# Lemok00/IDEAS

Hardware: AMD Instinct MI355X
Metric: train images/sec at 256x256 (G+D+Ex step) (higher is better)
Workload: dtype f32; 1 GPU; IDEAS N=1 sigma=1 256x256 batch=32/GPU full G+D+Ex iteration (lazy R1 every 16, EMA), full-width nets, HIP kernels (BASELINE.json configs[2]); global_batch=32, parallelism=dp1, r1_steps_in_window=0, ranks=1

## Files before the change

### ideas_amd/_lib.py

```python
from __future__ import annotations

import ctypes as C
import os
from typing import Optional

import torch

_HERE = os.path.dirname(os.path.abspath(__file__))
LIB_PATH = os.environ.get("IDEAS_HIP_LIB", os.path.join(_HERE, "libideas_hip.so"))

NCHW, NHWC = 0, 1
F32 = 0
F32_B3 = 1
BF16 = 2
F16 = 3
F64 = 4


def act_dtype(t: torch.Tensor) -> int:
    if t.dtype == torch.float32:
        return F32
    if t.dtype == torch.bfloat16:
        return BF16
    raise RuntimeError(f"ideas_amd: only float32 and bfloat16 activations are implemented, got {t.dtype}")
# ... 28 lines not shown
                ("block0", C.c_int), ("nblocks", C.c_int), ("pad_", C.c_int)]


PREP_B3_SPLIT, PREP_B3_WINO, PREP_BF16_PACK = 0, 1, 2


class LinearSeg(C.Structure):
    _fields_ = [("w", C.c_void_p), ("bias", C.c_void_p), ("y", C.c_void_p), ("gw", C.c_void_p), ("gb", C.c_void_p),
                ("n", C.c_int), ("ldw", C.c_int), ("ldy", C.c_int), ("ldgw", C.c_int), ("scale", C.c_float), ("bias_mul", C.c_float),
                ("tile0", C.c_int), ("pad_", C.c_int)]


LINEAR_MAX_SEGMENTS = 32
MBSTD_MAX_PARTIALS = 64
NOISE_ACT_MAX_PARTIALS = 2048
LPIPS_MAX_PARTIALS = 64
POOL_MAX_S2, POOL_MAX_S1P1, POOL_AVG_S1P1_VALID = 0, 1, 2
FEATURE_STATS_MAX_DIM = 4096
PATH_LERP, PATH_SLERP, PATH_MAX_DIM = 0, 1, 4096

_P = C.c_void_p
_PROTOS = {
    "ideas_abi_version": (C.c_int, []),
    "ideas_sizeof_conv_params": (C.c_int, []),
    "ideas_strerror": (C.c_char_p, [C.c_int]),
    "ideas_stream_create": (C.c_int, [C.POINTER(C.c_void_p), C.c_int]),
    "ideas_stream_destroy": (C.c_int, [_P]),
    "ideas_fused_bias_act": (C.c_int, [_P, _P, _P, _P, _P, C.c_int64, C.c_int, C.c_int64, C.c_int, C.c_int, C.c_int,
                                       C.c_float, C.c_float, C.c_int, _P]),
    "ideas_upfirdn2d": (C.c_int, [_P, _P, _P] + [C.c_int] * 14 + [C.c_float, C.c_int, C.c_int, C.c_int, _P]),
    "ideas_fir_up2_add": (C.c_int, [_P, _P, _P, _P] + [C.c_int] * 8 + [C.c_float, C.c_int, C.c_int, _P]),
    "ideas_blur_fused": (C.c_int, [_P, _P, _P] + [C.c_int] * 8 + [C.c_float, C.c_int, C.c_int, _P, _P, _P, C.c_float, C.c_float,
                                   C.c_int, _P]),
    "ideas_conv_igemm": (C.c_int, [_P, _P, _P, _P, _P, _P, _P, C.POINTER(ConvParams), C.c_int, _P]),
    "ideas_conv_igemm_multi": (C.c_int, [C.c_int, _P, _P, C.POINTER(C.c_void_p), _P, _P, C.POINTER(ConvParams), C.c_int, _P]),
    "ideas_b3_conv_supported": (C.c_int, [C.POINTER(ConvParams)]),
    "ideas_b3_wgrad_supported": (C.c_int, [C.POINTER(ConvParams)]),
    "ideas_b3_wgrad3_supported": (C.c_int, [C.POINTER(ConvParams)]),
    "ideas_b3_wino_supported": (C.c_int, [C.POINTER(ConvParams)]),
    "ideas_b3_wino_split_weights": (C.c_int, [_P, _P, C.c_int, C.c_int, C.c_int64, C.c_int64, C.c_int64, C.c_int64, C.c_int64, _P]),
    "ideas_b3_split_weights": (C.c_int, [_P, _P, C.c_int, C.c_int, C.c_int, _P]),
    "ideas_b3_split_weights_strided": (C.c_int, [_P, _P] + [C.c_int] * 4 + [C.c_int64] * 4 + [_P]),
    "ideas_bf16_conv_supported": (C.c_int, [C.POINTER(ConvParams), C.c_int]),
    "ideas_bf16_wgrad_supported": (C.c_int, [C.POINTER(ConvParams), C.c_int]),
    "ideas_bf16_direct_supported": (C.c_int, [C.POINTER(ConvParams)]),
    "ideas_bf16_pack_weights": (C.c_int, [_P, _P, _P, C.c_int, C.c_int, C.c_int, C.c_int, _P]),
    "ideas_bf16_pack_weights_strided": (C.c_int, [_P, _P, _P] + [C.c_int] * 5 + [C.c_int64] * 4 + [_P]),
    "ideas_conv3x3_wino": (C.c_int, [_P, _P, _P, _P, _P, _P, _P, C.POINTER(ConvParams), C.c_int, _P]),
    "ideas_conv3x3_wino_wgrad": (C.c_int, [_P, _P, _P, _P, _P, C.POINTER(ConvParams), C.c_int, _P]),
    "ideas_wino_wgrad_fold": (C.c_int, [_P, _P, C.c_int, C.c_int] + [C.c_int64] * 4 + [C.c_int, _P]),
    "ideas_b3_blur_conv_s2_supported": (C.c_int, [C.POINTER(ConvParams), C.c_int, C.c_int, C.c_int]),
    "ideas_b3_blur_conv_s2": (C.c_int, [_P, _P, _P, _P, C.POINTER(C.c_float), C.POINTER(C.c_float), _P, _P, C.POINTER(ConvParams),
                                        C.c_int, C.c_int, C.c_int, _P]),
    "ideas_b3_blur_conv_s2_mod": (C.c_int, [_P, _P, _P, _P, C.POINTER(C.c_float), C.POINTER(C.c_float), _P, _P, _P, _P,
                                            C.POINTER(ConvParams), C.c_int, C.c_int, C.c_int, _P]),
    "ideas_conv_direct": (C.c_int, [_P, _P, _P, _P, _P, _P, _P, C.POINTER(ConvParams), C.c_int, _P]),
    "ideas_conv_wgrad": (C.c_int, [_P, _P, _P, _P, _P, C.POINTER(ConvParams), C.c_int, _P]),
    "ideas_conv_wgrad_direct": (C.c_int, [_P, _P, _P, _P, _P, C.POINTER(ConvParams), C.c_int, _P]),
    "ideas_demod": (C.c_int, [_P, _P, _P, C.c_int, C.c_int, C.c_int, C.c_float, _P]),
    "ideas_weight_sqsum": (C.c_int, [_P, _P] + [C.c_int] * 4 + [C.c_int64] * 4 + [C.c_float, _P]),
    "ideas_weight_sqsum_f64": (C.c_int, [_P, _P] + [C.c_int] * 4 + [C.c_int64] * 4 + [C.c_double, _P]),
    "ideas_demod_bwd": (C.c_int, [_P] * 7 + [C.c_int] * 3 + [C.c_float, _P]),
    "ideas_demod_wgrad": (C.c_int, [_P] * 4 + [C.c_int] * 5 + [C.c_int64] * 8 + [C.c_float, _P]),
    "ideas_pixel_dot": (C.c_int, [_P, _P, _P, C.c_int, C.c_int64, C.c_int, C.c_int, _P]),
    "ideas_reflect_fold": (C.c_int, [_P, _P, C.c_int, C.c_int, C.c_int, C.c_int, C.c_int, C.c_int, _P]),
    "ideas_adam_ema": (C.c_int, [_P, _P, _P, _P, C.c_int64, C.c_float, C.c_float, C.c_float, C.c_float, C.c_float, _P]),
# ... 99 lines not shown
```

### ideas_amd/csrc/upfirdn2d.hip

```cpp
#include "common.hpp"

namespace {

struct FirParams {
    int B, C, in_h, in_w, out_h, out_w, kh, kw;
    int up_x, up_y, down_x, down_y, pad_x0, pad_y0;
    float gain;
    int flip;
    int seg_rows;
};

#define GENERIC_TAP_LDS 32768
template <bool NHWC, typename T, typename A, typename K>
__global__ __launch_bounds__(256) void upfirdn2d_generic(T* __restrict__ y, const T* __restrict__ x,
                                                         const K* __restrict__ fir, FirParams p, int lds_taps) {
    extern __shared__ double s_taps[];
    A* sk = reinterpret_cast<A*>(s_taps);
    if (lds_taps) {
        for (int t = threadIdx.x; t < p.kh * p.kw; t += blockDim.x) {
            int ky = t / p.kw, kx = t % p.kw;
            int src = p.flip ? (p.kh - 1 - ky) * p.kw + (p.kw - 1 - kx) : t;
            sk[t] = (A)fir[src] * (A)p.gain;
        }
        __syncthreads();
// ... 368 lines not shown
            if (t > 0) { hb.x = fmaf(v[t].x, kh[t - 1], hb.x); hb.y = fmaf(v[t].y, kh[t - 1], hb.y); hb.z = fmaf(v[t].z, kh[t - 1], hb.z); hb.w = fmaf(v[t].w, kh[t - 1], hb.w); }
        }
    };
    auto vsum = [&](const float4& r0, const float4& r1, const float4& r2, const float4& r3) {
        return make_float4(r0.x * kv[0] + r1.x * kv[1] + r2.x * kv[2] + r3.x * kv[3], r0.y * kv[0] + r1.y * kv[1] + r2.y * kv[2] + r3.y * kv[3],
                           r0.z * kv[0] + r1.z * kv[1] + r2.z * kv[2] + r3.z * kv[3], r0.w * kv[0] + r1.w * kv[1] + r2.w * kv[2] + r3.w * kv[3]);
    };
    float4 a0, a1, a2, a3, a4, b0, b1, b2, b3, b4;
    {
        const int iy0 = oy0 - p.pad_y0;
        hrow(iy0 + 0, a0, b0); hrow(iy0 + 1, a1, b1); hrow(iy0 + 2, a2, b2);
    }
    int oy = oy0;
#pragma unroll 1
    for (; oy + 1 < oy1; oy += 2) {
        hrow(oy - p.pad_y0 + 3, a3, b3);
        hrow(oy - p.pad_y0 + 4, a4, b4);
        fin(oy, 0, vsum(a0, a1, a2, a3));
        if (colB) fin(oy, 1, vsum(b0, b1, b2, b3));
        fin(oy + 1, 0, vsum(a1, a2, a3, a4));
        if (colB) fin(oy + 1, 1, vsum(b1, b2, b3, b4));
        a0 = a2; a1 = a3; a2 = a4; b0 = b2; b1 = b3; b2 = b4;
    }
    if (oy < oy1) {
        hrow(oy - p.pad_y0 + 3, a3, b3);
        fin(oy, 0, vsum(a0, a1, a2, a3));
        if (colB) fin(oy, 1, vsum(b0, b1, b2, b3));
    }
    if (EPI == EPI_ACT_BWD) {
        const float part[4] = {bsum.x, bsum.y, bsum.z, bsum.w};
        bgrad_flush(s_bg, ep.bgrad, p.C, active, 4 * c4, part, 4);
    }
}
template <int EPI, typename E>
__global__ __launch_bounds__(256) void blur4_bf16x8_c2(uint4* __restrict__ y, const uint4* __restrict__ x,
                                                       const float* __restrict__ fir, FirParams p, FirEpi ep) {
    __shared__ float sk[16];
    extern __shared__ float s_bg[];
    blur4_c2<VecX8<E>, EPI>(y, x, fir, p, ep, sk, s_bg);
}

template <typename T, int EPI>
__global__ __launch_bounds__(256) void blur4_nhwc(typename T::raw* __restrict__ y, const typename T::raw* __restrict__ x,
                                                  const float* __restrict__ fir, FirParams p, FirEpi ep) {
    typedef typename T::raw raw;
    constexpr int N = T::N;
    __shared__ float sk[16];
    extern __shared__ float s_bg[];
    stage_taps(sk, fir, p);
    const int CV = p.C >> T::SHIFT;
    Tile tl;
    const bool active = decode_tile(tl, p, CV, p.out_w, p.out_h);
    if (EPI != EPI_ACT_BWD && !active) return;
    const int ox = tl.col, oy0 = tl.r0, oy1 = tl.r1;
    const int ix0 = ox - p.pad_x0;
    float k[16];
#pragma unroll
    for (int t = 0; t < 16; ++t) k[t] = sk[t];
    const raw* xb = x + (int64_t)tl.b * p.in_h * p.in_w * CV + tl.cv;
    raw* yb = y + (((int64_t)tl.b * p.out_h) * p.out_w + ox) * CV + tl.cv;
    const raw* rb = reinterpret_cast<const raw*>(ep.ref) + (((int64_t)tl.b * p.out_h) * p.out_w + ox) * CV + tl.cv;
    float bb[N] = {}, bsum[N] = {};
    if (EPI == EPI_BIAS_ACT) {
#pragma unroll
        for (int e = 0; e < N; ++e) bb[e] = ep.bias[N * tl.cv + e];
    }
// ... 265 lines not shown
        }
    }
    if (dtype == IDEAS_BF16 && p.C % 8 == 0)
        FIR_LAUNCH((blur4_bf16x8_c2<EPI, ideas_bf16>), pairs * (p.C / 8), lds, stream, (uint4*)y, (const uint4*)x, fir, p, ep);
    else if (dtype == IDEAS_BF16)
        FIR_LAUNCH((blur4_nhwc<VecBf16x4, EPI>), total, lds, stream, (ideas_bf16x4*)y, (const ideas_bf16x4*)x, fir, p, ep);
    else
        FIR_LAUNCH(blur4_f32_c2<EPI>, pairs * (p.C / 4), lds, stream, (float4*)y, (const float4*)x, fir, p, ep);
    return ideas_launch_status();
}

static void launch_down2(void* y, const void* x, const float* fir, const FirParams& p, int64_t tiles, int dtype, bool x8, hipStream_t stream) {
    if (x8 && dtype == IDEAS_F16)
        FIR_LAUNCH(fir4_down2_bf16x8<_Float16>, tiles * (p.C / 8), 0, stream, (uint4*)y, (const uint4*)x, fir, p);
    else if (x8)
        FIR_LAUNCH(fir4_down2_bf16x8<ideas_bf16>, tiles * (p.C / 8), 0, stream, (uint4*)y, (const uint4*)x, fir, p);
    else if (dtype == IDEAS_BF16)
        FIR_LAUNCH(fir4_down2_nhwc<VecBf16x4>, tiles * (p.C / 4), 0, stream, (ideas_bf16x4*)y, (const ideas_bf16x4*)x, fir, p);
    else
        FIR_LAUNCH(fir4_down2_nhwc<VecF32>, tiles * (p.C / 4), 0, stream, (float4*)y, (const float4*)x, fir, p);
}
static void launch_up2(void* y, const void* x, const float* fir, const FirParams& p, const void* resid, int64_t tiles, int dtype, bool x8,
                       hipStream_t stream) {
    if (x8 && dtype == IDEAS_F16)
        FIR_LAUNCH(fir4_up2<VecX8<_Float16>>, tiles * (p.C / 8), 0, stream, (uint4*)y, (const uint4*)x, fir, p, (const uint4*)resid);
    else if (x8)
        FIR_LAUNCH(fir4_up2<VecX8<ideas_bf16>>, tiles * (p.C / 8), 0, stream, (uint4*)y, (const uint4*)x, fir, p, (const uint4*)resid);
    else if (dtype == IDEAS_BF16)
        FIR_LAUNCH(fir4_up2<VecBf16x4>, tiles * (p.C / 4), 0, stream, (ideas_bf16x4*)y, (const ideas_bf16x4*)x, fir, p, (const ideas_bf16x4*)resid);
    else
        FIR_LAUNCH(fir4_up2<VecF32>, tiles * (p.C / 4), 0, stream, (float4*)y, (const float4*)x, fir, p, (const float4*)resid);
}

#undef FIR_LAUNCH

extern "C" int ideas_blur_fused(void* y, const void* x, const float* fir, int B, int C, int in_h, int in_w, int out_h, int out_w,
                                int pad_x0, int pad_y0, float gain, int flip, int mode, const void* ref, const float* bias,
                                float* bias_grad, float alpha, float scale, int dtype, void* stream_) {
    if (dtype != IDEAS_F32 && dtype != IDEAS_BF16) return IDEAS_E_UNSUPPORTED;
    if (!y || !x || !fir) return IDEAS_E_NULL;
    if (B <= 0 || C <= 0 || in_h <= 0 || in_w <= 0 || out_h <= 0 || out_w <= 0) return IDEAS_E_SHAPE;
    if (C % 4 || C > 8192) return IDEAS_E_UNSUPPORTED;
    if (!ideas_aligned16(x) || !ideas_aligned16(y)) return IDEAS_E_ALIGN;
    FirParams p{B, C, in_h, in_w, out_h, out_w, 4, 4, 1, 1, 1, 1, pad_x0, pad_y0, gain, flip, 16};
    FirEpi ep{ref, bias, bias_grad, alpha, scale};
    hipStream_t stream = (hipStream_t)stream_;
    if (mode == EPI_ACT_BWD) {
        if (!ref || !bias_grad) return IDEAS_E_NULL;
        if (!ideas_aligned16(ref)) return IDEAS_E_ALIGN;
        return launch_blur4<EPI_ACT_BWD>(y, x, fir, p, ep, dtype, stream);
    }
    if (mode == EPI_BIAS_ACT) {
        if (!bias) return IDEAS_E_NULL;
        if (!ideas_aligned16(bias)) return IDEAS_E_ALIGN;
        return launch_blur4<EPI_BIAS_ACT>(y, x, fir, p, ep, dtype, stream);
    }
    return IDEAS_E_UNSUPPORTED;
}

static int upfirdn2d_impl(void* y, const void* x, const float* fir, int B, int C, int in_h, int in_w, int out_h,
                          int out_w, int kh, int kw, int up_x, int up_y, int down_x, int down_y, int pad_x0,
                          int pad_y0, float gain, int flip, int layout, int dtype, void* stream_, const void* resid) {
    if (dtype != IDEAS_F32 && dtype != IDEAS_BF16 && dtype != IDEAS_F16 && dtype != IDEAS_F64) return IDEAS_E_UNSUPPORTED;
    if (dtype == IDEAS_BF16 && layout != IDEAS_NHWC) return IDEAS_E_UNSUPPORTED;
    if (!y || !x || !fir) return IDEAS_E_NULL;
    if (B <= 0 || C <= 0 || in_h <= 0 || in_w <= 0 || out_h <= 0 || out_w <= 0) return IDEAS_E_SHAPE;
    if (kh <= 0 || kw <= 0) return IDEAS_E_UNSUPPORTED;
// ... 85 lines not shown
```

### ideas_amd/op/modulated_conv.py

```python
from __future__ import annotations

import math
from typing import Optional

import torch
from torch.autograd import Function
from torch.autograd.function import once_differentiable

from .. import _lib
from ..precision import to_act, to_f32
from . import conv as _conv
from .conv import conv2d, conv_dgrad_raw, conv_fwd_raw, conv_transpose2d, conv_wgrad_raw, _nhwc
from .conv_plan import ConvGeom, convT_out_size
from . import conv_plan
from . import scratch
from .upfirdn2d import _geometry, blur_bias_act, blur_pads, upfirdn2d, upfirdn2d_raw
from .fused_act import bias_sink, fused_leaky_relu
from .grad_sink import weight_grad


def pixel_dot(a: torch.Tensor, g: torch.Tensor) -> torch.Tensor:
    a, g = _nhwc(a), _nhwc(g)
    b, c, h, w = a.shape
    out = scratch.zeros((b, c), a.device, torch.float64)
    if a.dtype != g.dtype:
        a, g = a.float(), g.float()
    if a.dtype == torch.bfloat16 and c % 4:
        a, g = a.float(), g.float()
    rc = _lib.load().ideas_pixel_dot(_lib.ptr(out), _lib.ptr(a), _lib.ptr(g), b, h * w, c, _lib.act_dtype(a), _lib.stream_ptr())
    _lib.check(rc, "ideas_pixel_dot")
    return out


def _weight_sqsum(w: torch.Tensor, scale: float, dtype, entry: str, key: str) -> torch.Tensor:
    def make():
        cout, cin, kh, kw = w.shape
        wsq = torch.empty((cout, cin), device=w.device, dtype=dtype)
        _lib.check(getattr(_lib.load(), entry)(_lib.ptr(wsq), _lib.ptr(w), cout, cin, kh, kw, *w.stride(), float(scale * scale),
                                               _lib.stream_ptr()), entry)
        return wsq
    return conv_plan.cached(w, (key, float(scale)), make)


def weight_sqsum(w: torch.Tensor, scale: float) -> torch.Tensor:
    return _weight_sqsum(w, scale, torch.float32, "ideas_weight_sqsum", "wsq")


def weight_sqsum_f64(w: torch.Tensor, scale: float) -> torch.Tensor:
    return _weight_sqsum(w, scale, torch.float64, "ideas_weight_sqsum_f64", "wsq64")
# ... 24 lines not shown
    cout = w.shape[0]
    if dot_s.dtype != torch.float64 or (dot_d is not None and dot_d.dtype != torch.float64):
        raise RuntimeError("_style_grads takes the float64 accumulators of pixel_dot / act_bwd_dot")
    if d is not None:
        gq, wsq = torch.empty_like(d), weight_sqsum_f64(w, gain)
    rc = _lib.load().ideas_demod_bwd(_lib.ptr(gs), _lib.ptr(gq), _lib.ptr(dot_s), _lib.ptr(dot_d), _lib.ptr(d), _lib.ptr(s),
                                     _lib.ptr(wsq), b, cin, cout, float(eps), _lib.stream_ptr())
    _lib.check(rc, "ideas_demod_bwd")
    return gs, gq


def _demod_wgrad(gw: torch.Tensor, w: torch.Tensor, gq: torch.Tensor, s: torch.Tensor, gain: float) -> None:
    cout, cin, kh, kw = w.shape
    rc = _lib.load().ideas_demod_wgrad(_lib.ptr(gw), _lib.ptr(w), _lib.ptr(gq), _lib.ptr(s), s.shape[0], cout, cin, kh, kw,
                                       *w.stride(), *gw.stride(), float(2.0 * gain * gain), _lib.stream_ptr())
    _lib.check(rc, "ideas_demod_wgrad")


def act_bwd_dot(gy: torch.Tensor, out: torch.Tensor, bias: torch.Tensor, alpha: float, act_gain: float, bias_grad_into=None):
    gy, out = _nhwc(gy), _nhwc(out)
    if gy.dtype != out.dtype:
        gy = gy.to(out.dtype)
    b, c, h, w = out.shape
    gpre = torch.empty_like(out)
    bg = bias_grad_into if bias_grad_into is not None else torch.zeros(c, device=out.device, dtype=torch.float32)
    dot = scratch.zeros((b, c), out.device, torch.float64)
    rc = _lib.load().ideas_act_bwd_dot(_lib.ptr(gpre), _lib.ptr(bg), _lib.ptr(dot), _lib.ptr(gy), _lib.ptr(out),
                                       _lib.ptr(bias), None, b, h * w, c, float(alpha), float(act_gain), _lib.act_dtype(out),
                                       _lib.stream_ptr())
    _lib.check(rc, "ideas_act_bwd_dot")
    return gpre, (None if bias_grad_into is not None else bg), dot


def _mod_geom(mode: str, k: int) -> ConvGeom:
    if mode == "same":
        return ConvGeom(k, k, 1, k // 2, False)
    return ConvGeom(k, k, 1 if (mode == "down" and k == 1) else 2, 0, False)


def _down_blur(x, fir, k: int, pad2):
    down = 2 if k == 1 else 1
    return (down,) + _geometry((x.shape[2], x.shape[3]), fir, 1, down, pad2)


def _mod_forward(x, w, s, d, mode: str, fir, pad2, gain: float, bias=None, slope: float = 0.2, act_gain: float = 1.0, resid=None,
                 want_xb: bool = False):
    k = w.shape[2]
    g = _mod_geom(mode, k)
    epi = dict(lin=s, lout=d, bias=bias, act=bias is not None, act_gain=act_gain, alpha=slope)
    if mode == "same":
        return conv_fwd_raw(x, w, g, gain, resid=resid, **epi), None
    if mode == "up":
        return conv_dgrad_raw(x, w.transpose(0, 1), g, convT_out_size(x.shape[2], x.shape[3], g), gain, lin=s, lout=d), None
    if k == 3 and _conv.mod_blur_conv_ok(x, w, fir, pad2, want_xb=want_xb):
        return _conv.blur_conv_s2_raw(x, w, fir, pad2, gain, want_xb=want_xb, **epi)
    down, pad4, bhw, _ = _down_blur(x, fir, k, pad2)
    xb = upfirdn2d_raw(x, fir, (1, 1), (down, down), pad4, bhw, flip=True)
    return conv_fwd_raw(xb, w, g, gain, **epi), xb


class _ModConv(Function):

    @staticmethod
    def forward(ctx, x, w, s, b, mode: str, fir, pad2, gain: float, demod: bool, eps: float, slope: float, act_gain: float):
        x = _nhwc(x)
        s = s.contiguous()
        ctx.bias_ref = b
        if b is not None:
            b = b.contiguous()
        d = demod_of(w, s, gain, eps) if demod else None
        need_w = ctx.needs_input_grad[1]
        y, xb = _mod_forward(x, w, s, d, mode, fir, pad2, gain, b, slope, act_gain, want_xb=need_w)
        ctx.mode, ctx.pad2, ctx.gain, ctx.eps, ctx.slope, ctx.act_gain = mode, pad2, gain, eps, slope, act_gain
        keep = dict(x=x, w=w, s=s, fir=fir, d=d, b=b,
                    y=y if (b is not None or d is not None) else None,
                    xb=xb if need_w else None)
        ctx.names = [n for n, t in keep.items() if t is not None]
        ctx.save_for_backward(*(keep[n] for n in ctx.names))
        return y

    @staticmethod
    @once_differentiable
    def backward(ctx, gy):
        t = dict(zip(ctx.names, ctx.saved_tensors))
        x, w, s, d, b, y = t["x"], t["w"], t["s"], t.get("d"), t.get("b"), t.get("y")
        mode, gain = ctx.mode, ctx.gain
        g = _mod_geom(mode, w.shape[2])
        need_x, need_w, need_s, need_b = ctx.needs_input_grad[:4]
        gb = dot_d = None
        if b is not None:
            gpre, gb, dot_d = act_bwd_dot(gy, y, b, ctx.slope, ctx.act_gain, bias_grad_into=bias_sink(ctx.bias_ref) if need_b else None)
        else:
            gpre = gy = _nhwc(gy)
        gx = gw = gs = gq = None
        if need_x or need_s:
            if mode == "up":
                gx = conv_fwd_raw(gpre, w.transpose(0, 1), g, gain, lin=d, lout=s)
            elif mode == "same":
                gx = conv_dgrad_raw(gpre, w, g, (x.shape[2], x.shape[3]), gain, lin=d, lout=s)
            else:
                down, _, bhw, g_pad = _down_blur(x, t["fir"], w.shape[2], ctx.pad2)
                gx = conv_dgrad_raw(gpre, w, g, bhw, gain, lin=d, lout=s)
                gx = upfirdn2d_raw(gx, t["fir"], (down, down), (1, 1), g_pad, (x.shape[2], x.shape[3]), flip=False)
        if need_s or (need_w and d is not None):
            dot_s = pixel_dot(x, gx) if need_s else scratch.zeros(tuple(s.shape), s.device, torch.float64)
            if d is not None and dot_d is None:
                dot_d = pixel_dot(gy, y)
            gs, gq = _style_grads(dot_s, dot_d, s, d, w, gain, ctx.eps)
        if need_w:
            xin = t["xb"] if mode == "down" else x

            def grad(out):
                if mode == "up":
                    r = conv_wgrad_raw(xin, gpre, g, (w.shape[1], w.shape[0], w.shape[2], w.shape[3]), gain, lin=d, lout=s,
                                       out=None if out is None else out.transpose(0, 1)).transpose(0, 1)
                else:
                    r = conv_wgrad_raw(gpre, xin, g, tuple(w.shape), gain, lin=s, lout=d, out=out)
                if gq is not None:
                    _demod_wgrad(r, w, gq, s, gain)
                return r
            gw = weight_grad(w, grad, gpre, xin, s, d, gq)
        return ((gx if need_x else None), gw, (gs if need_s else None), (gb if need_b else None),
                None, None, None, None, None, None, None, None)
# ... 35 lines not shown


def modulated_conv2d(x: torch.Tensor, weight: torch.Tensor, style: torch.Tensor, demodulate: bool = True,
                     upsample: bool = False, fir: Optional[torch.Tensor] = None, eps: float = 1e-8,
                     act_bias: Optional[torch.Tensor] = None, negative_slope: float = 0.2,
                     act_scale: float = 2 ** 0.5, resid: Optional[torch.Tensor] = None, downsample: bool = False) -> torch.Tensor:
    if upsample and downsample:
        raise ValueError("modulated_conv2d: upsample and downsample are exclusive")
    _lib.require_cuda(x, weight, style)
    mode = "down" if downsample else "up" if upsample else "same"
    if mode != "same" and fir is None:
        raise RuntimeError(f"modulated_conv2d({mode}sample=True) needs the blur FIR")
    if downsample:
        if resid is not None:
            raise RuntimeError("modulated_conv2d(resid=...) is the no-grad fast path of the fused same-resolution conv")
        _lib.require_cuda(fir, act_bias)
    x, style = to_act(x), to_f32(style)
    if resid is not None:
        resid = to_act(resid)
    w = weight[0] if weight.dim() == 5 else weight
    cout, cin, k, _ = w.shape
    if _SECOND_ORDER[0] and torch.is_grad_enabled() and resid is None:
        return _modulated_conv2d_composite(x, w, style, demodulate, upsample, fir, eps, act_bias, negative_slope, act_scale, downsample)
    scale = 1.0 / math.sqrt(cin * k * k)
    pad2 = blur_pads(fir.shape[0], k, up=upsample) if mode != "same" else None
    fuse_act = act_bias is not None and not upsample and demodulate and cout % 4 == 0
    if resid is not None:
        if not fuse_act or torch.is_grad_enabled():
            raise RuntimeError("modulated_conv2d(resid=...) is the no-grad fast path of the fused same-resolution conv")
        style = style.contiguous()
        d = demod_raw(style, weight_sqsum(w, scale), eps)
        return _mod_forward(x, w, style, d, mode, None, None, scale, act_bias.contiguous(), float(negative_slope), float(act_scale),
                            resid=resid)[0]
    y = _ModConv.apply(x, w, style, act_bias if fuse_act else None, mode, *((fir, pad2) if downsample else (None, None)),
                       scale, bool(demodulate), float(eps), float(negative_slope), float(act_scale))
    if upsample:
        if act_bias is not None:
            return blur_bias_act(y, fir, pad2, act_bias, negative_slope, act_scale)
        return upfirdn2d(y, fir, pad=pad2)
    if act_bias is not None and not fuse_act:
        y = fused_leaky_relu(y, act_bias, negative_slope, act_scale)
    return y
```

### ideas_amd/op/upfirdn2d.py

```python
from __future__ import annotations

from typing import Tuple

import torch
from torch.autograd import Function

from .. import _lib


def upfirdn2d_raw(x: torch.Tensor, fir: torch.Tensor, up: Tuple[int, int], down: Tuple[int, int],
                  pad: Tuple[int, int, int, int], out_hw: Tuple[int, int], flip: bool, gain: float = 1.0) -> torch.Tensor:
    _lib.require_cuda(x, fir)
    dt = _lib.op_dtype(x)
    if x.dim() != 4:
        raise RuntimeError("upfirdn2d expects a 4-D [B, C, H, W] tensor")
    lib = _lib.load()
    b, c, h, w = x.shape
    kh, kw = fir.shape
    oh, ow = out_hw
    if oh <= 0 or ow <= 0:
        raise RuntimeError(f"upfirdn2d: empty output {oh}x{ow}")
    if x.is_contiguous(memory_format=torch.channels_last):
        layout, fmt = _lib.NHWC, torch.channels_last
    elif x.is_contiguous() and dt != _lib.BF16:
# ... 10 lines not shown
    return y


BLUR_ACT_BWD, BLUR_BIAS_ACT = 1, 2


def blur_fused_ok(x: torch.Tensor, fir: torch.Tensor) -> bool:
    return (x.dim() == 4 and x.is_cuda and x.dtype in (torch.float32, torch.bfloat16) and x.shape[1] % 4 == 0 and tuple(fir.shape) == (4, 4)
            and x.is_contiguous(memory_format=torch.channels_last))


def blur_fused_raw(x: torch.Tensor, fir: torch.Tensor, pad: Tuple[int, int, int, int], out_hw: Tuple[int, int], flip: bool,
                   mode: int, ref=None, bias=None, bias_grad=None, alpha: float = 0.2, scale: float = 1.0) -> torch.Tensor:
    _lib.require_cuda(x, fir, ref, bias, bias_grad)
    b, c, h, w = x.shape
    oh, ow = out_hw
    x = x if x.is_contiguous(memory_format=torch.channels_last) else x.contiguous(memory_format=torch.channels_last)
    if ref is not None:
        if tuple(ref.shape) != (b, c, oh, ow):
            raise RuntimeError("blur_fused: ref shape mismatch")
        if ref.dtype != x.dtype:
            x = x.to(ref.dtype)
        ref = ref if ref.is_contiguous(memory_format=torch.channels_last) else ref.contiguous(memory_format=torch.channels_last)
    if bias is not None:
        bias = bias.contiguous().to(torch.float32)
    y = torch.empty((b, c, oh, ow), device=x.device, dtype=x.dtype, memory_format=torch.channels_last)
    rc = _lib.load().ideas_blur_fused(_lib.ptr(y), _lib.ptr(x), _lib.ptr(fir.contiguous().to(torch.float32)), b, c, h, w, oh, ow,
                                      pad[0], pad[2], 1.0, int(flip), mode, _lib.ptr(ref), _lib.ptr(bias), _lib.ptr(bias_grad),
                                      float(alpha), float(scale), _lib.act_dtype(x), _lib.stream_ptr())
    _lib.check(rc, "ideas_blur_fused")
    return y


def blur_geometry(in_hw: Tuple[int, int], fir: torch.Tensor, pad2: Tuple[int, int]):
    return _geometry(in_hw, fir, 1, 1, pad2)


class _BlurBiasAct(Function):

    @staticmethod
    def forward(ctx, x, fir, pad2, bias, slope: float, scale: float):
        pad4, out_hw, g_pad = blur_geometry((x.shape[2], x.shape[3]), fir, pad2)
        out = blur_fused_raw(x, fir, pad4, out_hw, True, BLUR_BIAS_ACT, bias=bias, alpha=slope, scale=scale)
        ctx.pad4, ctx.g_pad, ctx.in_size, ctx.out_hw, ctx.slope, ctx.scale = pad4, g_pad, tuple(x.shape), out_hw, slope, scale
        ctx.bias_ref = bias
        ctx.save_for_backward(out, fir)
        return out

    @staticmethod
    def backward(ctx, gy):
        from .fused_act import FusedLeakyReLUFunctionBackward, bias_act_raw, bias_sink
        out, fir = ctx.saved_tensors
        one = (1, 1)
        tgt = bias_sink(ctx.bias_ref) if ctx.needs_input_grad[3] else None
        if tgt is not None:
            g_pre, gb = bias_act_raw(gy, None, out, 1, ctx.slope, ctx.scale, bias_grad_into=tgt)
        else:
            g_pre, gb = FusedLeakyReLUFunctionBackward.apply(gy, out, ctx.slope, ctx.scale, True)
        gx = None
        if ctx.needs_input_grad[0]:
            gx = UpFirDn2dBackward.apply(g_pre, fir, one, one, ctx.pad4, ctx.g_pad, ctx.in_size, ctx.out_hw)
        return gx, None, None, (gb if (ctx.needs_input_grad[3] and tgt is None) else None), None, None


def blur_bias_act(x: torch.Tensor, fir: torch.Tensor, pad, bias: torch.Tensor, negative_slope: float = 0.2,
                  scale: float = 2 ** 0.5) -> torch.Tensor:
# ... 139 lines not shown
```

### include/ideas_hip.h

```cpp
#ifndef IDEAS_HIP_H
#define IDEAS_HIP_H

#include <stdint.h>

#ifdef __cplusplus
extern "C" {
#endif

#define IDEAS_ABI_VERSION 4

enum { IDEAS_NCHW = 0, IDEAS_NHWC = 1 };
enum { IDEAS_F32 = 0, IDEAS_F32_B3 = 1, IDEAS_BF16 = 2, IDEAS_F16 = 3, IDEAS_F64 = 4 };

enum {
    IDEAS_OK = 0,
    IDEAS_E_NULL = -1,
    IDEAS_E_SHAPE = -2,
    IDEAS_E_UNSUPPORTED = -3,
    IDEAS_E_ALIGN = -4
};

int ideas_abi_version(void);
int ideas_sizeof_conv_params(void);
const char* ideas_strerror(int code);

int ideas_stream_create(void** out_stream, int prio);
int ideas_stream_destroy(void* stream);

int ideas_fused_bias_act(void* y, const void* x, const void* b, const void* ref, float* bias_grad,
                         int64_t n, int C, int64_t inner, int layout,
                         int act, int grad, float alpha, float scale, int dtype, void* stream);

int ideas_channel_sum(float* out, const void* x, int64_t n, int C, int clear, int dtype, void* stream);

int ideas_upfirdn2d(void* y, const void* x, const float* fir,
                    int B, int C, int in_h, int in_w, int out_h, int out_w,
                    int kh, int kw, int up_x, int up_y, int down_x, int down_y,
                    int pad_x0, int pad_y0, float gain, int flip,
                    int layout, int dtype, void* stream);

int ideas_fir_up2_add(void* y, const void* x, const float* fir, const void* resid, int B, int C, int in_h, int in_w, int out_h,
                      int out_w, int pad_x0, int pad_y0, float gain, int flip, int dtype, void* stream);

#define IDEAS_BLUR_ACT_BWD 1
#define IDEAS_BLUR_BIAS_ACT 2
int ideas_blur_fused(void* y, const void* x, const float* fir, int B, int C, int in_h, int in_w, int out_h, int out_w,
                     int pad_x0, int pad_y0, float gain, int flip, int mode, const void* ref, const float* bias,
                     float* bias_grad, float alpha, float scale, int dtype, void* stream);

typedef struct ideas_conv_params {
    int B, IH, IW, Cin;
    int YH, YW, Cout;
    int OH, OW;
    int TY, TX;
    int sy, sx, dy, dx, offy, offx;
    int osy, osx, ooy, oox;
    int reflect;
    int act;
    float alpha, act_gain, resid_gain;
    int accumulate;
    float gain;
} ideas_conv_params;

int ideas_conv_igemm(void* y, const void* x, const void* wmat, const float* in_scale, const float* out_scale,
                     const float* bias, const void* resid, const ideas_conv_params* p, int dtype, void* stream);

int ideas_b3_conv_supported(const ideas_conv_params* p);
int ideas_b3_wgrad_supported(const ideas_conv_params* p);
int ideas_b3_wgrad3_supported(const ideas_conv_params* p);
int ideas_b3_split_weights(void* planes, const void* wmat, int Cout, int K, int Cin, void* stream);
int ideas_b3_split_weights_strided(void* planes, const float* w, int Cout, int TY, int TX, int Cin, int64_t sn, int64_t sty,
                                   int64_t stx, int64_t sc, void* stream);
int ideas_b3_wino_supported(const ideas_conv_params* p);
int ideas_b3_wino_split_weights(void* planes, const void* w, int N, int C, int64_t sn, int64_t sky, int64_t skx, int64_t sc,
                                int64_t base, void* stream);

int ideas_bf16_conv_supported(const ideas_conv_params* p, int scaled);
int ideas_bf16_wgrad_supported(const ideas_conv_params* p, int scaled);
int ideas_bf16_pack_weights(void* pack, const void* wmat, const float* in_scale, int B, int Cout, int K, int Cin, void* stream);
int ideas_bf16_pack_weights_strided(void* pack, const float* w, const float* in_scale, int B, int Cout, int TY, int TX, int Cin,
                                    int64_t sn, int64_t sty, int64_t stx, int64_t sc, void* stream);
// ... 154 lines not shown
```

Baseline: 81.50 images/sec.

## Fuse upsample modconv blur+bias-act backward with activation grad and demod dot

Result: no change. 82.15 images/sec (median of 6 runs) (+0.8%).

```diff
diff --git a/ideas_amd/_lib.py b/ideas_amd/_lib.py
--- a/ideas_amd/_lib.py
+++ b/ideas_amd/_lib.py
@@ -84,6 +84,7 @@
     "ideas_fir_up2_add": (C.c_int, [_P, _P, _P, _P] + [C.c_int] * 8 + [C.c_float, C.c_int, C.c_int, _P]),
     "ideas_blur_fused": (C.c_int, [_P, _P, _P] + [C.c_int] * 8 + [C.c_float, C.c_int, C.c_int, _P, _P, _P, C.c_float, C.c_float,
                                    C.c_int, _P]),
+    "ideas_act_bwd_blur": (C.c_int, [_P] * 7 + [C.c_int] * 8 + [C.c_float, C.c_float, C.c_int, _P]),
     "ideas_conv_igemm": (C.c_int, [_P, _P, _P, _P, _P, _P, _P, C.POINTER(ConvParams), C.c_int, _P]),
     "ideas_conv_igemm_multi": (C.c_int, [C.c_int, _P, _P, C.POINTER(C.c_void_p), _P, _P, C.POINTER(ConvParams), C.c_int, _P]),
     "ideas_b3_conv_supported": (C.c_int, [C.POINTER(ConvParams)]),
diff --git a/ideas_amd/csrc/upfirdn2d.hip b/ideas_amd/csrc/upfirdn2d.hip
--- a/ideas_amd/csrc/upfirdn2d.hip
+++ b/ideas_amd/csrc/upfirdn2d.hip
@@ -424,6 +424,156 @@
         bgrad_flush(s_bg, ep.bgrad, p.C, active, 4 * c4, part, 4);
     }
 }
+#define ACT_BLUR_SLOTS 2
+template <int PX>
+__global__ __launch_bounds__(256) void act_bwd_blur4_f32(float4* __restrict__ y, const float4* __restrict__ gy, const float4* __restrict__ ref,
+                                                         const float* __restrict__ fir, const float* __restrict__ bias,
+                                                         float* __restrict__ bgrad, double* __restrict__ dot, FirParams p, float alpha,
+                                                         float scale) {
+    __shared__ float sk[16];
+    extern __shared__ double s_red[];
+    double* s_dot = s_red;
+    float* s_bg = reinterpret_cast<float*>(s_red + ACT_BLUR_SLOTS * p.C);
+    for (int c = threadIdx.x; c < ACT_BLUR_SLOTS * p.C; c += blockDim.x) s_dot[c] = 0.0;
+    for (int c = threadIdx.x; c < p.C; c += blockDim.x) s_bg[c] = 0.f;
+    stage_taps(sk, fir, p);
+    float kh[4], kv[4];
+    const bool sep = factor_taps(sk, kh, kv);
+    const int C4 = p.C >> 2;
+    const int cols = (p.out_w + 1) >> 1;
+    Tile tl;
+    const bool active = decode_tile(tl, p, C4, cols, p.out_h);
+    const int c4 = tl.cv, b = tl.b, oy0 = tl.r0, oy1 = tl.r1;
+    const int b_first = (int)(((int64_t)blockIdx.x * blockDim.x) / ((int64_t)((p.out_h + p.seg_rows - 1) / p.seg_rows) * cols * C4));
+    const int ox = 2 * tl.col;
+    const bool colB = ox + 1 < p.out_w;
+    const int ix0 = ox - PX;
+    const float4 zero = make_float4(0.f, 0.f, 0.f, 0.f);
+    const float4* gb = gy + (int64_t)b * p.in_h * p.in_w * C4 + c4;
+    const float4* rb = ref + (int64_t)b * p.in_h * p.in_w * C4 + c4;
+    float4* yb = y + (((int64_t)b * p.out_h) * p.out_w + ox) * C4 + c4;
+    const float4 bb = bias ? *reinterpret_cast<const float4*>(bias + 4 * c4) : zero;
+    const float inv_gain = 1.0f / scale, inv_alpha = 1.0f / alpha;
+    float4 bsum = zero;
+    struct { double x, y, z, w; } dacc = {0.0, 0.0, 0.0, 0.0};
+    auto gpre = [&](const float4& g, const float4& o) {
+        return make_float4(epi_act(g.x, o.x, alpha, scale), epi_act(g.y, o.y, alpha, scale), epi_act(g.z, o.z, alpha, scale),
+                           epi_act(g.w, o.w, alpha, scale));
+    };
+    auto reduce = [&](const float4& gp, const float4& o) {
+        bsum.x += gp.x; bsum.y += gp.y; bsum.z += gp.z; bsum.w += gp.w;
+        if (dot) {
+#define ONE(f)                                                                    \
+    {                                                                             \
+        const float t = o.f * inv_gain;                                           \
+        const float pre = ((t > 0.f) ? t : t * inv_alpha) - bb.f;                 \
+        dacc.f = fma((double)gp.f, (double)pre, dacc.f);                          \
+    }
+            ONE(x) ONE(y) ONE(z) ONE(w)
+#undef ONE
+        }
+    };
+    auto flush = [&]() {
+        if (active) {
+            if (bgrad) { atomicAdd(&s_bg[4 * c4 + 0], bsum.x); atomicAdd(&s_bg[4 * c4 + 1], bsum.y); atomicAdd(&s_bg[4 * c4 + 2], bsum.z); atomicAdd(&s_bg[4 * c4 + 3], bsum.w); }
+            if (dot) {
+                const int slot = b - b_first;
+                double* d = slot < ACT_BLUR_SLOTS ? s_dot + slot * p.C + 4 * c4 : dot + (int64_t)b * p.C + 4 * c4;
+                atomicAdd(d + 0, dacc.x); atomicAdd(d + 1, dacc.y); atomicAdd(d + 2, dacc.z); atomicAdd(d + 3, dacc.w);
+            }
+        }
+        __syncthreads();
+        if (bgrad)
+            for (int c = threadIdx.x; c < p.C; c += blockDim.x) {
+                const float v = s_bg[c];
+                if (v != 0.f) atomicAdd(&bgrad[c], v);
+            }
+        if (dot)
+            for (int c = threadIdx.x; c < ACT_BLUR_SLOTS * p.C; c += blockDim.x) {
+                const double v = s_dot[c];
+                const int bs = b_first + c / p.C;
+                if (v != 0.0 && bs < p.B) atomicAdd(&dot[(int64_t)bs * p.C + c % p.C], v);
+            }
+    };
+    const unsigned colmask = col_mask<5>(ix0, p.in_w);
+    if (!sep) {
+#pragma unroll 1
+        for (int oy = oy0; oy < oy1; ++oy)
+#pragma unroll 1
+            for (int col = 0; col < (colB ? 2 : 1); ++col) {
+                float4 acc = zero;
+#pragma unroll 1
+                for (int j = 0; j < 4; ++j) {
+                    const int iy = oy - p.pad_y0 + j;
+                    if (iy < 0 || iy >= p.in_h) continue;
+#pragma unroll 1
+                    for (int t = 0; t < 4; ++t) {
+                        const int ix = ix0 + col + t;
+                        if (ix < 0 || ix >= p.in_w) continue;
+                        const int64_t off = ((int64_t)iy * p.in_w + ix) * C4;
+                        const float4 v = gpre(gb[off], rb[off]);
+                        const float kk = sk[4 * j + t];
+                        acc.x = fmaf(v.x, kk, acc.x); acc.y = fmaf(v.y, kk, acc.y); acc.z = fmaf(v.z, kk, acc.z); acc.w = fmaf(v.w, kk, acc.w);
+                    }
+                }
+                if (active) yb[(int64_t)oy * p.out_w * C4 + (int64_t)col * C4] = acc;
+                if (active && oy < p.in_h && ox + col < p.in_w) {
+                    const int64_t off = ((int64_t)oy * p.in_w + ox + col) * C4;
+                    const float4 o = rb[off];
+                    reduce(gpre(gb[off], o), o);
+                }
+            }
+        flush();
+        return;
+    }
+    auto hrow = [&](int iy, float4& ha, float4& hb) {
+        const bool rowok = (iy >= 0) && (iy < p.in_h);
+        const int64_t roff = (int64_t)(rowok ? iy : 0) * p.in_w * C4;
+        float4 v[5], o[5];
+#pragma unroll
+        for (int t = 0; t < 5; ++t) {
+            const bool ok = rowok && ((colmask >> t) & 1u);
+            const int64_t off = roff + (int64_t)(ok ? ix0 + t : 0) * C4;
+            v[t] = gb[off];
+            o[t] = rb[off];
+        }
+#pragma unroll
+        for (int t = 0; t < 5; ++t) {
+            const bool ok = rowok && ((colmask >> t) & 1u);
+            const float4 w = gpre(v[t], o[t]);
+            v[t] = make_float4(ok ? w.x : 0.f, ok ? w.y : 0.f, ok ? w.z : 0.f, ok ? w.w : 0.f);
+        }
+        ha = zero; hb = zero;
+#pragma unroll
+        for (int t = 0; t < 5; ++t) {
+            if (t < 4) { ha.x = fmaf(v[t].x, kh[t], ha.x); ha.y = fmaf(v[t].y, kh[t], ha.y); ha.z = fmaf(v[t].z, kh[t], ha.z); ha.w = fmaf(v[t].w, kh[t], ha.w); }
+            if (t > 0) { hb.x = fmaf(v[t].x, kh[t - 1], hb.x); hb.y = fmaf(v[t].y, kh[t - 1], hb.y); hb.z = fmaf(v[t].z, kh[t - 1], hb.z); hb.w = fmaf(v[t].w, kh[t - 1], hb.w); }
+        }
+        if (active && rowok && iy >= oy0 && iy < oy1) {
+            if ((colmask >> PX) & 1u) reduce(v[PX], o[PX]);
+            if ((colmask >> (PX + 1)) & 1u) reduce(v[PX + 1], o[PX + 1]);
+        }
+    };
+    auto vsum = [&](const float4& r0, const float4& r1, const float4& r2, const float4& r3) {
+        return make_float4(dot4(r0.x, r1.x, r2.x, r3.x, kv[0], kv[1], kv[2], kv[3]), dot4(r0.y, r1.y, r2.y, r3.y, kv[0], kv[1], kv[2], kv[3]),
+                           dot4(r0.z, r1.z, r2.z, r3.z, kv[0], kv[1], kv[2], kv[3]), dot4(r0.w, r1.w, r2.w, r3.w, kv[0], kv[1], kv[2], kv[3]));
+    };
+    auto fin = [&](int oy, int col, const float4& acc) {
+        if (active) yb[(int64_t)oy * p.out_w * C4 + (int64_t)col * C4] = acc;
+    };
+    float4 a0, a1, a2, a3, b0, b1, b2, b3;
+    {
+        const int iy0 = oy0 - p.pad_y0;
+        hrow(iy0 + 0, a0, b0); hrow(iy0 + 1, a1, b1); hrow(iy0 + 2, a2, b2);
+    }
+    for (int oy = oy0; oy < oy1; ++oy) {
+        hrow(oy - p.pad_y0 + 3, a3, b3);
+        fin(oy, 0, vsum(a0, a1, a2, a3));
+        if (colB) fin(oy, 1, vsum(b0, b1, b2, b3));
+        a0 = a1; a1 = a2; a2 = a3; b0 = b1; b1 = b2; b2 = b3;
+    }
+    flush();
+}
 template <int EPI, typename E>
 __global__ __launch_bounds__(256) void blur4_bf16x8_c2(uint4* __restrict__ y, const uint4* __restrict__ x,
                                                        const float* __restrict__ fir, FirParams p, FirEpi ep) {
@@ -755,7 +905,38 @@
         FIR_LAUNCH(fir4_up2<VecF32>, tiles * (p.C / 4), 0, stream, (float4*)y, (const float4*)x, fir, p, (const float4*)resid);
 }
 
+static int launch_act_bwd_blur(float4* y, const float4* gy, const float4* ref, const float* fir, const float* bias, float* bgrad, double* dot,
+                               FirParams p, float alpha, float scale, hipStream_t stream) {
+    p.seg_rows = 16;
+    const int segs = (p.out_h + p.seg_rows - 1) / p.seg_rows;
+    const int64_t total = (int64_t)p.B * segs * ((p.out_w + 1) / 2) * (p.C / 4);
+    if (ideas_cdiv(total, 256) > 0x7fffffffLL) return IDEAS_E_SHAPE;
+    const size_t lds = (size_t)p.C * (ACT_BLUR_SLOTS * sizeof(double) + sizeof(float));
+    switch (p.pad_x0) {
+    case 0: FIR_LAUNCH(act_bwd_blur4_f32<0>, total, lds, stream, y, gy, ref, fir, bias, bgrad, dot, p, alpha, scale); break;
+    case 1: FIR_LAUNCH(act_bwd_blur4_f32<1>, total, lds, stream, y, gy, ref, fir, bias, bgrad, dot, p, alpha, scale); break;
+    case 2: FIR_LAUNCH(act_bwd_blur4_f32<2>, total, lds, stream, y, gy, ref, fir, bias, bgrad, dot, p, alpha, scale); break;
+    default: FIR_LAUNCH(act_bwd_blur4_f32<3>, total, lds, stream, y, gy, ref, fir, bias, bgrad, dot, p, alpha, scale); break;
+    }
+    return ideas_launch_status();
+}
+
 #undef FIR_LAUNCH
+
+extern "C" int ideas_act_bwd_blur(void* gx, float* bias_grad, double* dot, const void* gy, const void* out, const float* bias,
+                                  const float* fir, int B, int C, int H, int W, int GH, int GW, int pad_x0, int pad_y0, float alpha,
+                                  float act_gain, int dtype, void* stream_) {
+    if (dtype != IDEAS_F32) return IDEAS_E_UNSUPPORTED;
+    if (!gx || !gy || !out || !fir) return IDEAS_E_NULL;
+    if (B <= 0 || C <= 0 || H <= 0 || W <= 0 || GH <= 0 || GW <= 0) return IDEAS_E_SHAPE;
+    if (C % 4 || C > 2048) return IDEAS_E_UNSUPPORTED;
+    if (GH < H || GW < W || pad_x0 < 0 || pad_x0 > 3 || pad_y0 < 0 || pad_y0 > 3) return IDEAS_E_UNSUPPORTED;
+    if (dot && (alpha == 0.f || act_gain == 0.f)) return IDEAS_E_UNSUPPORTED;
+    if (!ideas_aligned16(gx) || !ideas_aligned16(gy) || !ideas_aligned16(out) || (bias && !ideas_aligned16(bias))) return IDEAS_E_ALIGN;
+    FirParams p{B, C, H, W, GH, GW, 4, 4, 1, 1, 1, 1, pad_x0, pad_y0, 1.f, 0, 16};
+    return launch_act_bwd_blur((float4*)gx, (const float4*)gy, (const float4*)out, fir, bias, bias_grad, dot, p, alpha, act_gain,
+                               (hipStream_t)stream_);
+}
 
 extern "C" int ideas_blur_fused(void* y, const void* x, const float* fir, int B, int C, int in_h, int in_w, int out_h, int out_w,
                                 int pad_x0, int pad_y0, float gain, int flip, int mode, const void* ref, const float* bias,
diff --git a/ideas_amd/op/modulated_conv.py b/ideas_amd/op/modulated_conv.py
--- a/ideas_amd/op/modulated_conv.py
+++ b/ideas_amd/op/modulated_conv.py
@@ -1,6 +1,7 @@
 from __future__ import annotations
 
 import math
+import os
 from typing import Optional
 
 import torch
@@ -14,7 +15,8 @@
 from .conv_plan import ConvGeom, convT_out_size
 from . import conv_plan
 from . import scratch
-from .upfirdn2d import _geometry, blur_bias_act, blur_pads, upfirdn2d, upfirdn2d_raw
+from .upfirdn2d import (BLUR_BIAS_ACT, _geometry, act_bwd_blur_blocks, act_bwd_blur_raw, blur_bias_act, blur_fused_raw, blur_geometry,
+                        blur_pads, upfirdn2d, upfirdn2d_raw)
 from .fused_act import bias_sink, fused_leaky_relu
 from .grad_sink import weight_grad
 
@@ -105,6 +107,20 @@
     return gpre, (None if bias_grad_into is not None else bg), dot
 
 
+UP_BWD_MIN_BLOCKS = 512
+
+
+def up_bwd_fused_ok(x: torch.Tensor, w: torch.Tensor, fir, demodulate: bool, act_bias) -> bool:
+    if os.environ.get("IDEAS_UP_BWD_FUSED", "1") == "0":
+        return False
+    cout, k = w.shape[0], w.shape[2]
+    if not (x.dtype == torch.float32 and cout % 4 == 0 and cout <= 2048 and demodulate and act_bias is not None and fir is not None
+            and tuple(fir.shape) == (4, 4) and k == 3):
+        return False
+    gh, gw = convT_out_size(x.shape[2], x.shape[3], _mod_geom("up", k))
+    return act_bwd_blur_blocks(x.shape[0], cout, gh, gw) >= UP_BWD_MIN_BLOCKS
+
+
 def _mod_geom(mode: str, k: int) -> ConvGeom:
     if mode == "same":
         return ConvGeom(k, k, 1, k // 2, False)
@@ -124,7 +140,11 @@
     if mode == "same":
         return conv_fwd_raw(x, w, g, gain, resid=resid, **epi), None
     if mode == "up":
-        return conv_dgrad_raw(x, w.transpose(0, 1), g, convT_out_size(x.shape[2], x.shape[3], g), gain, lin=s, lout=d), None
+        y = conv_dgrad_raw(x, w.transpose(0, 1), g, convT_out_size(x.shape[2], x.shape[3], g), gain, lin=s, lout=d)
+        if bias is not None:
+            pad4, out_hw, _ = blur_geometry((y.shape[2], y.shape[3]), fir, pad2)
+            y = blur_fused_raw(y, fir, pad4, out_hw, True, BLUR_BIAS_ACT, bias=bias, alpha=slope, scale=act_gain)
+        return y, None
     if k == 3 and _conv.mod_blur_conv_ok(x, w, fir, pad2, want_xb=want_xb):
         return _conv.blur_conv_s2_raw(x, w, fir, pad2, gain, want_xb=want_xb, **epi)
     down, pad4, bhw, _ = _down_blur(x, fir, k, pad2)
@@ -161,7 +181,14 @@
         g = _mod_geom(mode, w.shape[2])
         need_x, need_w, need_s, need_b = ctx.needs_input_grad[:4]
         gb = dot_d = None
-        if b is not None:
+        if b is not None and mode == "up":
+            _, _, g_pad = blur_geometry(convT_out_size(x.shape[2], x.shape[3], g), t["fir"], ctx.pad2)
+            sink = bias_sink(ctx.bias_ref) if need_b else None
+            gb = torch.zeros_like(b, dtype=torch.float32) if (need_b and sink is None) else None
+            dot_d = scratch.zeros((y.shape[0], y.shape[1]), y.device, torch.float64) if d is not None else None
+            gpre = act_bwd_blur_raw(_nhwc(gy), y, b, t["fir"], g_pad, convT_out_size(x.shape[2], x.shape[3], g), ctx.slope, ctx.act_gain,
+                                    bias_grad=sink if sink is not None else gb, dot=dot_d)
+        elif b is not None:
             gpre, gb, dot_d = act_bwd_dot(gy, y, b, ctx.slope, ctx.act_gain, bias_grad_into=bias_sink(ctx.bias_ref) if need_b else None)
         else:
             gpre = gy = _nhwc(gy)
@@ -263,8 +290,14 @@
         d = demod_raw(style, weight_sqsum(w, scale), eps)
         return _mod_forward(x, w, style, d, mode, None, None, scale, act_bias.contiguous(), float(negative_slope), float(act_scale),
                             resid=resid)[0]
-    y = _ModConv.apply(x, w, style, act_bias if fuse_act else None, mode, *((fir, pad2) if downsample else (None, None)),
+    fuse_up = upsample and up_bwd_fused_ok(x, w, fir, demodulate, act_bias)
+    if fuse_up:
+        _lib.require_cuda(fir, act_bias)
+    y = _ModConv.apply(x, w, style, act_bias if (fuse_act or fuse_up) else None, mode,
+                       *((fir, pad2) if (downsample or fuse_up) else (None, None)),
                        scale, bool(demodulate), float(eps), float(negative_slope), float(act_scale))
+    if fuse_up:
+        return y
     if upsample:
         if act_bias is not None:
             return blur_bias_act(y, fir, pad2, act_bias, negative_slope, act_scale)
diff --git a/ideas_amd/op/upfirdn2d.py b/ideas_amd/op/upfirdn2d.py
--- a/ideas_amd/op/upfirdn2d.py
+++ b/ideas_amd/op/upfirdn2d.py
@@ -66,6 +66,31 @@
     return y
 
 
+def act_bwd_blur_blocks(b: int, c: int, gh: int, gw: int) -> int:
+    return -(-(b * -(-gh // 16) * ((gw + 1) // 2) * (c // 4)) // 256)
+
+
+def act_bwd_blur_raw(gy: torch.Tensor, out: torch.Tensor, bias, fir: torch.Tensor, g_pad: Tuple[int, int, int, int],
+                     gx_hw: Tuple[int, int], alpha: float, scale: float, bias_grad=None, dot=None) -> torch.Tensor:
+    _lib.require_cuda(gy, out, bias, fir, bias_grad, dot)
+    cl = torch.channels_last
+    b, c, h, w = out.shape
+    if tuple(gy.shape) != tuple(out.shape) or tuple(fir.shape) != (4, 4):
+        raise RuntimeError("act_bwd_blur: gy / out shape mismatch or a FIR that is not 4x4")
+    if gy.dtype != out.dtype:
+        gy = gy.to(out.dtype)
+    gy = gy if gy.is_contiguous(memory_format=cl) else gy.contiguous(memory_format=cl)
+    out = out if out.is_contiguous(memory_format=cl) else out.contiguous(memory_format=cl)
+    if bias is not None:
+        bias = bias.contiguous().to(torch.float32)
+    gx = torch.empty((b, c, gx_hw[0], gx_hw[1]), device=out.device, dtype=out.dtype, memory_format=cl)
+    rc = _lib.load().ideas_act_bwd_blur(_lib.ptr(gx), _lib.ptr(bias_grad), _lib.ptr(dot), _lib.ptr(gy), _lib.ptr(out), _lib.ptr(bias),
+                                        _lib.ptr(fir.contiguous().to(torch.float32)), b, c, h, w, gx_hw[0], gx_hw[1], g_pad[0], g_pad[2],
+                                        float(alpha), float(scale), _lib.act_dtype(out), _lib.stream_ptr())
+    _lib.check(rc, "ideas_act_bwd_blur")
+    return gx
+
+
 def blur_geometry(in_hw: Tuple[int, int], fir: torch.Tensor, pad2: Tuple[int, int]):
     return _geometry(in_hw, fir, 1, 1, pad2)
 
diff --git a/include/ideas_hip.h b/include/ideas_hip.h
--- a/include/ideas_hip.h
+++ b/include/ideas_hip.h
@@ -47,6 +47,10 @@
 int ideas_blur_fused(void* y, const void* x, const float* fir, int B, int C, int in_h, int in_w, int out_h, int out_w,
                      int pad_x0, int pad_y0, float gain, int flip, int mode, const void* ref, const float* bias,
                      float* bias_grad, float alpha, float scale, int dtype, void* stream);
+
+int ideas_act_bwd_blur(void* gx, float* bias_grad, double* dot, const void* gy, const void* out, const float* bias, const float* fir,
+                       int B, int C, int H, int W, int GH, int GW, int pad_x0, int pad_y0, float alpha, float act_gain, int dtype,
+                       void* stream);
 
 typedef struct ideas_conv_params {
     int B, IH, IW, Cin;
```
